# mmaker/c-lwe-snarks

Hardware: AMD Instinct MI355X
Metric: snark_proofs_per_sec (higher is better)
Workload: dtype u32 limbs (704-bit integers mod 2^704) + AES-256 bytes; int8 digits on the matrix cores, int32 accumulation (exact)

## Files before the change

c-lwe-snarks_amd/__init__.py:

```python
from __future__ import annotations

import ctypes
import os
from dataclasses import dataclass

import numpy as np

_HERE = os.path.dirname(os.path.abspath(__file__))
LIB_PATH = os.environ.get("MFHIP_LIB") or os.path.join(_HERE, "libmfhip.so")
P = 0xFFFFFFFB


class MfhError(RuntimeError):
    pass


@dataclass(frozen=True)
class Params:

    n: int = 1470
    logq: int = 736
    d: int = 1 << 15
    m: int = 21845

# ... 51 lines not shown
EXPORTS = [
    "mfh_ctx_create", "mfh_ctx_destroy", "mfh_set_stream", "mfh_sync", "mfh_scrub_staging", "mfh_last_error", "mfh_set_seed",
    "mfh_keystream", "mfh_sample_rows", "mfh_ct_add", "mfh_ct_mul_ui", "mfh_ct_addmul_ui", "mfh_eval_rows",
    "mfh_encrypt_rows", "mfh_decrypt", "mfh_ct_smudge", "mfh_ssp_upload", "mfh_witness_poly", "mfh_version",
    "mfh_workspace_bytes", "mfh_last_kernel_ms", "mfh_set_timing", "mfh_set_overlap", "mfh_eval_rows_multi", "mfh_prove_batch", "mfh_crs_mm_image_bytes", "mfh_crs_expand_mm", "mfh_crs_set_resident_mm", "mfh_witness_poly_multi", "mfh_witness_poly_mm", "mfh_poly_h_multi", "mfh_poly_mul", "mfh_poly_add", "mfh_poly_prepare_t",
    "mfh_ssp_prepare", "mfh_poly_h", "mfh_setup_messages", "mfh_setup", "mfh_setup_image", "mfh_crs_image_set_b", "mfh_prove",
    "mfh_prove_partial", "mfh_prove_finish", "mfh_ct_to_lanes", "mfh_ct_from_lanes", "mfh_lanes_per_value", "mfh_digest128", "mfh_timing_drain", "mfh_timing_busy_ms", "mfh_timing_work_rows", "mfh_set_batch_image", "mfh_set_batch_slabs", "mfh_set_expand_path", "mfh_set_expand_periods", "mfh_set_encrypt_path", "mfh_set_batch_launch", "mfh_set_batch_bw", "mfh_set_batch_witness", "mfh_witness_poly_stream", "mfh_set_mm_chunk_rows", "mfh_set_mm_pack", "mfh_set_poly_exact", "mfh_poly_exact_fallbacks", "mfh_poly_exact_points", "mfh_set_poly_exact_points", "mfh_set_mm_stream", "mfh_add_dotp", "mfh_set_encrypt_chunks", "mfh_set_witness_per", "mfh_set_eval_path", "mfh_set_decrypt_path", "mfh_decrypt_rows",
    "mfh_crs_mm_share_bytes", "mfh_crs_expand_mm_share", "mfh_crs_set_resident_mm_share", "mfh_batch_chain", "mfh_batch_witness_cols", "mfh_batch_chain_from_w", "mfh_witness_poly_mm_cols", "mfh_prove_batch_partial", "mfh_prove_batch_finish",
    "mfh_resident_row_bytes", "mfh_crs_expand", "mfh_eval_rows_resident", "mfh_crs_set_resident",
    "mfh_witness_lanes", "mfh_witness_from_lanes", "mfh_prove_partial_w", "mfh_verify",
    "mfh_ssp_set_prg", "mfh_ssp_prg_make_t", "mfh_ssp_prg_fill",
    "mfh_resident_share_rows", "mfh_crs_expand_share", "mfh_crs_set_resident_share", "mfh_crs_set_resident_prefix",
    "mfh_prove_batch_supergroup", "mfh_prove_batch_stream_wait", "mfh_set_mm_width", "mfh_set_mm_queue", "mfh_set_mm_claim_log", "mfh_mm_claim_log_launches",
    "mfh_setup_public", "mfh_prove_public", "mfh_prove_batch_public", "mfh_vk_derive", "mfh_verify_public",
    "mfh_ssp_from_rows", "mfh_ssp_set_rows", "mfh_ssp_rows_fill", "mfh_ssp_rows_violations", "mfh_circuit_create", "mfh_circuit_destroy", "mfh_circuit_assign",
    "mfh_circuit_create_global", "mfh_circuit_create_ex", "mfh_circuit_create_out", "mfh_circuit_create_sum",
    "mfh_merkle_create", "mfh_merkle_destroy", "mfh_merkle_set_leaves", "mfh_merkle_root", "mfh_merkle_nodes", "mfh_merkle_paths",
    "mfh_sha256_records", "mfh_merkle_set_records", "mfh_merkle_update_rows", "mfh_merkle_update_records",
    "mfh_merkle_absent_rows", "mfh_merkle_insert_keys", "mfh_merkle_update_rows_cut", "mfh_merkle_update_records_cut", "mfh_merkle_insert_keys_cut",
    "mfh_merkle_remove_keys", "mfh_merkle_remove_keys_cut", "mfh_merkle_transfer_keys", "mfh_merkle_transfer_keys_cut",
    "mfh_merkle_paths_cut", "mfh_merkle_absent_rows_cut", "mfh_merkle_range_rows", "mfh_merkle_range_rows_cut",
    "mfh_merkle_load_keys", "mfh_merkle_check_table", "mfh_merkle_grow", "mfh_merkle_grow_leaves",
    "mfh_merkle_write_keys", "mfh_merkle_write_keys_cut",
]


OPTIONAL_EXPORTS = {
    "mfh_set_mm_queue": "tuning knob; older builds walk fixed lists",
    "mfh_set_mm_claim_log": "test instrumentation of mfh_set_mm_queue",
    "mfh_mm_claim_log_launches": "test instrumentation of mfh_set_mm_queue",
    "mfh_set_expand_periods": "test knob; older builds pick the periods per chunk from the row count",
    "mfh_set_batch_witness": "tuning knob; older builds run the witness pass per super-group",
    "mfh_witness_poly_stream": "the streamed pass alone (tests); older builds have mfh_witness_poly_mm only",
}


def load_library():
    global _lib
    if _lib is not None:
        return _lib
    if not os.path.exists(LIB_PATH):
        raise MfhError(f"{LIB_PATH} is missing: run `python -c 'import __graft_entry__ as g; g.build()'` "
                       "(hipcc --offload-arch=gfx950).  There is no CPU fallback.")
    lib = ctypes.CDLL(LIB_PATH)
    vp, u64, sz, i32, u32 = ctypes.c_void_p, ctypes.c_uint64, ctypes.c_size_t, ctypes.c_int, ctypes.c_uint32
    sig = {
        "mfh_ctx_create": (i32, [ctypes.POINTER(vp), i32, ctypes.POINTER(_CParams)]),
        "mfh_ctx_destroy": (None, [vp]),
        "mfh_set_stream": (i32, [vp, vp]),
        "mfh_sync": (i32, [vp]),
        "mfh_scrub_staging": (i32, [vp]),
        "mfh_last_error": (ctypes.c_char_p, [vp]),
        "mfh_set_seed": (i32, [vp, ctypes.c_char_p]),
        "mfh_keystream": (i32, [vp, u64, vp, sz]),
        "mfh_sample_rows": (i32, [vp, u64, sz, vp]),
        "mfh_ct_add": (i32, [vp, vp, vp, vp, sz]),
# ... 48 lines not shown
        "mfh_ssp_set_prg": (i32, [vp, u64, vp]),
        "mfh_ssp_prg_make_t": (i32, [vp, u64, ctypes.c_char_p, vp]),
        "mfh_ssp_prg_fill": (i32, [vp, u64, sz, sz, vp]),
        "mfh_verify": (i32, [vp, vp, u32, u32, u32, vp, vp, sz, vp]),
        "mfh_witness_lanes": (i32, [vp, vp, ctypes.c_char_p, u32, u32, vp]),
        "mfh_witness_from_lanes": (i32, [vp, vp, vp, u32, vp]),
        "mfh_prove_partial_w": (i32, [vp, vp, vp, ctypes.c_char_p, u32, u32, u32, vp, vp]),
        "mfh_resident_row_bytes": (sz, [vp]),
        "mfh_crs_expand": (i32, [vp, u64, sz, vp, vp]),
        "mfh_crs_image_set_b": (i32, [vp, sz, sz, vp, vp]),
        "mfh_eval_rows_resident": (i32, [vp, vp, sz, sz, vp, vp, vp, vp, i32]),
        "mfh_crs_set_resident": (i32, [vp, vp]),
        "mfh_timing_drain": (i32, [vp, ctypes.c_char_p, ctypes.POINTER(u64), ctypes.POINTER(ctypes.c_double), ctypes.POINTER(u64),
                                   ctypes.POINTER(ctypes.c_float)]),
        "mfh_timing_busy_ms": (ctypes.c_double, [vp]),
        "mfh_timing_work_rows": (u64, [vp]),
        "mfh_set_batch_image": (i32, [vp, i32]),
        "mfh_set_mm_chunk_rows": (i32, [vp, u32]),
        "mfh_set_mm_pack": (i32, [vp, i32]),
        "mfh_set_poly_exact": (i32, [vp, i32]),
        "mfh_poly_exact_fallbacks": (ctypes.c_long, [vp]),
        "mfh_poly_exact_points": (i32, [vp, ctypes.POINTER(u32)]),
        "mfh_set_poly_exact_points": (i32, [vp, ctypes.POINTER(u32)]),
        "mfh_set_mm_stream": (i32, [vp, i32, i32, i32, u32]),
        "mfh_set_batch_launch": (i32, [vp, u32, i32]),
        "mfh_set_batch_bw": (i32, [vp, i32]),
        "mfh_set_batch_witness": (i32, [vp, i32]),
        "mfh_set_encrypt_path": (i32, [vp, i32]),
        "mfh_set_expand_path": (i32, [vp, i32]),
        "mfh_set_expand_periods": (i32, [vp, u32]),
        "mfh_set_batch_slabs": (i32, [vp, u32]),
        "mfh_set_encrypt_chunks": (i32, [vp, u32]),
        "mfh_set_eval_path": (i32, [vp, i32]),
        "mfh_set_decrypt_path": (i32, [vp, i32]),
        "mfh_decrypt_rows": (i32, [vp, u64, sz, vp, vp, vp]),
        "mfh_set_witness_per": (i32, [vp, u32]),
        "mfh_crs_mm_share_bytes": (sz, [vp, u32, u32]),
        "mfh_crs_expand_mm_share": (i32, [vp, vp, u32, u32, vp]),
        "mfh_crs_set_resident_mm_share": (i32, [vp, vp, u32, u32]),
        "mfh_batch_chain": (i32, [vp, vp, u32, ctypes.c_char_p, sz, vp, vp, vp, vp]),
        "mfh_batch_witness_cols": (i32, [vp, vp, u32, ctypes.c_char_p, sz, vp, u32, u32, vp, sz]),
        "mfh_batch_chain_from_w": (i32, [vp, vp, u32, vp, vp, vp]),
        "mfh_witness_poly_mm_cols": (i32, [vp, vp, u32, ctypes.c_char_p, sz, vp, u32, u32, vp, sz]),
        "mfh_prove_batch_partial": (i32, [vp, vp, u32, u32, u32, ctypes.c_char_p, sz, vp, vp, vp, sz, vp]),
        "mfh_prove_batch_finish": (i32, [vp, vp, u32, vp, ctypes.c_char_p, sz, ctypes.c_char_p, vp]),
        "mfh_setup_public": (i32, [vp, vp, u32, u32, u32, u32, vp, vp, vp, vp]),
# ... 951 lines not shown
    def set_mm_pack(self, on=True):
        self._chk(self.lib.mfh_set_mm_pack(self._h, 1 if on else 0))

    def set_poly_exact(self, mode=1):
        self._chk(self.lib.mfh_set_poly_exact(self._h, int(mode)))

    def poly_exact_fallbacks(self):
        return int(self.lib.mfh_poly_exact_fallbacks(self._h))

    def exact_points(self):
        out = (ctypes.c_uint32 * 4)()
        self._chk(self.lib.mfh_poly_exact_points(self._h, out))
        return [int(x) for x in out]

    def set_exact_points(self, pts):
        if pts is None:
            self._chk(self.lib.mfh_set_poly_exact_points(self._h, None))
            return
        pts = [int(x) for x in pts]
        if len(pts) != 4 or not all(0 <= x < 2**32 for x in pts):
            raise MfhError(f"set_exact_points: four uint32 values, got {pts!r}")
        self._chk(self.lib.mfh_set_poly_exact_points(self._h, (ctypes.c_uint32 * 4)(*pts)))

    def set_mm_chunk_rows(self, rows=0):
        self._chk(self.lib.mfh_set_mm_chunk_rows(self._h, int(rows)))

    def timing_drain(self, which):
        n, rows, ms, last = ctypes.c_uint64(), ctypes.c_uint64(), ctypes.c_double(), ctypes.c_float()
        self._chk(self.lib.mfh_timing_drain(self._h, which.encode(), ctypes.byref(n), ctypes.byref(ms), ctypes.byref(rows), ctypes.byref(last)))
        return n.value, ms.value, rows.value

    def timing_busy_ms(self):
        return float(self.lib.mfh_timing_busy_ms(self._h))

    def timing_work_rows(self):
        return int(self.lib.mfh_timing_work_rows(self._h))

    def last_kernel_ms(self, which):
        return float(self.lib.mfh_last_kernel_ms(self._h, which.encode()))

    def set_seed(self, seed: bytes):
        assert len(seed) == 40
        self._chk(self.lib.mfh_set_seed(self._h, bytes(seed)))

    def keystream(self, off, nbytes, out=None):
        out = self.empty(nbytes) if out is None else out
# ... 467 lines not shown
```

c-lwe-snarks_amd/csrc/ctx.hpp:

```cpp
#pragma once
#include <hip/hip_runtime.h>

#include <stdint.h>
#include <string.h>

#include <string>
#include <vector>

#include "aes_dev.hpp"
#include "batch_plan.hpp"
#include "mfhip.h"
#include "ssp_prg.hpp"

#define HIP_TRY(ctx, expr)                                                        \
  do {                                                                            \
    hipError_t e_ = (expr);                                                       \
    if (e_ != hipSuccess) {                                                       \
      (ctx)->err = std::string(#expr) + ": " + hipGetErrorString(e_);             \
      return MFH_EDEVICE;                                                         \
    }                                                                             \
  } while (0)

struct PolyState;
struct SspInterp;
// ... 65 lines not shown
  const uint32_t *ssp_frag_src = nullptr;
  DevBuf ssp_img;
  const uint32_t *ssp_img_src = nullptr;
  DevBuf wstream;
  hipEvent_t ev_wstage = nullptr, ev_wdigits = nullptr;
  int batch_witness = 1;
  SspInterp *interp = nullptr;
  DevBuf circ_io;
  DevBuf circ_state;
  DevBuf d_batch;
  DevBuf batch_img;
  int batch_image = 1;
  int mm_map = 1;
  bool mm_persist = true;
  bool mm_wave1 = false;
  uint32_t mm_sync_mode = 0, mm_spin = 64;
  uint32_t mm_width = 32;
  size_t early_ws_half = 0;
  bool batch_early_chain = false;
  uint32_t *mm_sync = nullptr;
  uint32_t mm_queue = 1, mm_queue_shift = 0; int mm_queue_prefix = -8;
  uint32_t *mm_log = nullptr; size_t mm_log_words = 0, mm_log_used = 0; uint32_t mm_log_n = 0, mm_log_desc[16][12];
  int poly_exact = 1;
  bool poly_pts_pinned = false;
  uint32_t poly_pts[4] = {0, 0, 0, 0};
  bool mm_pack = true;
  uint32_t mm_chunk_rows = 131071;
  int expand_path = 0;
  uint32_t expand_periods = 0;
  int enc_path = 0;
  uint32_t ncu = 256;
  int dec_path = 0;
  int eval_path = 0;
  uint32_t enc_chunks = 0;
  uint32_t witness_per = 0;
  uint32_t batch_slabs = 0;
  int batch_bw_merged = 1;
  int batch_merge = 1;
  uint32_t batch_ngl = 8;
  PinBuf pin_rows, pin_cw, pin_smudge;
  PinBuf pin_pub;
  DevBuf d_pub;
  PinBuf pin_wring[8];
  uint32_t pin_wnext = 0;
  hipEvent_t ev_sample = nullptr;
  DevBuf sample_tmp;
// ... 223 lines not shown
```

c-lwe-snarks_amd/csrc/poly.hip:

```cpp
#include <assert.h>
#include <errno.h>
#include <sys/syscall.h>
#include <unistd.h>

#include <algorithm>
#include <type_traits>

#include "ctx.hpp"
#include "ntt.hpp"

namespace {

#define MF_NEEDED(need, vs) do { if ((need) && (vs) >= *(need)) return; } while (0)

using namespace mf_ntt;

__device__ __forceinline__ uint32_t lz_mont(uint32_t a, uint32_t b, uint32_t p, uint32_t ninv) {
  uint64_t t = (uint64_t)a * b;
  uint32_t m = (uint32_t)t * ninv;
  return (uint32_t)((t + (uint64_t)m * p) >> 32);
}
__device__ __forceinline__ uint32_t lz_add(uint32_t a, uint32_t b, uint32_t p2) {
  uint32_t s = a + b;
  return min(s, s - p2);
// ... 282 lines not shown
#pragma unroll
  for (int m = 0; m < 8; m++) sm[lpad(8 * tid + m)] = v[m];
  __syncthreads();
#pragma unroll
  for (int m = 0; m < 8; m++) v[m] = sm[lpad(i3 + 4 * m)];
  dit_regs<3, true>(v, j3, 4, 8, ti, half_max, q);
#pragma unroll
  for (int m = 0; m < 8; m++) sm[lpad(i3 + 4 * m)] = v[m];
  __syncthreads();
#pragma unroll
  for (int m = 0; m < 8; m++) v[m] = sm[lpad(i2 + 32 * m)];
  dit_regs<3, true>(v, j2, 32, 64, ti, half_max, q);
#pragma unroll
  for (int m = 0; m < 8; m++) sm[lpad(i2 + 32 * m)] = v[m];
  __syncthreads();
#pragma unroll
  for (int m = 0; m < 8; m++) v[m] = sm[lpad(i1 + 256 * m)];
  dit_regs<3, true>(v, tid, 256, 512, ti, half_max, q);
#pragma unroll
  for (int m = 0; m < 8; m++) a[base + i1 + 256 * m] = lz_canon(v[m], q.p);
}

__global__ void k_crt(const uint32_t *__restrict__ r, uint32_t N, uint32_t count, Primes3 P, Crt C, uint32_t *__restrict__ out, size_t out_stride,
                      const uint32_t *__restrict__ need = nullptr, int64_t rev_top = -1, uint32_t nsrc = 0, const uint32_t *__restrict__ map = nullptr) {
  MF_NEEDED(need, blockIdx.y);
  uint32_t i = blockIdx.x * blockDim.x + threadIdx.x;
  if (i >= count) return;
  r += (size_t)blockIdx.y * 3 * N;
  out += (size_t)(map ? map[blockIdx.y] : blockIdx.y) * out_stride;
  if (rev_top < 0) {
    out[i] = crt_coeff(r[i], r[(size_t)N + i], r[(size_t)2 * N + i], P, C);
    return;
  }
  const int64_t e = rev_top - (int64_t)i;
  out[i] = e >= 0 && e < (int64_t)nsrc ? crt_coeff(r[e], r[(size_t)N + e], r[(size_t)2 * N + e], P, C) : 0u;
}
template <int K, bool LAST>
__global__ __launch_bounds__(256) void k_exact_seam(uint32_t *__restrict__ a, uint32_t N, const uint32_t *__restrict__ tw, const uint32_t *__restrict__ twi,
                                                    uint32_t half_max, Primes3 P, Crt C, uint32_t *__restrict__ out, uint32_t keep, size_t out_stride) {
  constexpr int R = 1 << K;
  constexpr uint32_t qd = 2048;
  const uint32_t j = blockIdx.x * blockDim.x + threadIdx.x;
  if (j >= qd || N != (qd << K)) return;
  uint32_t *x = a + (size_t)blockIdx.y * 3 * N + j;
  const NttPrime q1 = P.q[0], q2 = P.q[1], q3 = P.q[2];
  uint32_t r[R], x1[R], x2[R], cf[R];
#pragma unroll
  for (int m = 0; m < R; m++) r[m] = x[(size_t)m * qd];
  dit_regs<K>(r, j, qd, 2 * qd, twi, half_max, q1);
#pragma unroll
  for (int m = 0; m < R; m++) x1[m] = mont_mul(r[m], C.ninv_std[0], q1.p, q1.ninv);
  __builtin_amdgcn_sched_barrier(0);
#pragma unroll
  for (int m = 0; m < R; m++) r[m] = x[(size_t)N + (size_t)m * qd];
// ... 13 lines not shown
    const uint32_t x1m3 = x1[m] >= q3.p ? x1[m] - q3.p : x1[m], x2m3 = x2[m] >= q3.p ? x2[m] - q3.p : x2[m];
    const uint32_t t3 = mont_mul(sub_mod(r3, x1m3, q3.p), C.inv_p1_p3, q3.p, q3.ninv);
    const uint32_t x3 = mont_mul(sub_mod(t3, x2m3, q3.p), C.inv_p2_p3, q3.p, q3.ninv);
    cf[m] = red_p32((uint64_t)red_p32(x1[m]) + red_p32((uint64_t)x2[m] * C.p1_mod) + red_p32((uint64_t)x3 * C.p1p2_mod));
  }
  if (LAST) {
    out += (size_t)blockIdx.y * out_stride;
#pragma unroll
    for (int m = 0; m < R; m++)
      if (j + (uint32_t)m * qd < keep) out[j + (uint32_t)m * qd] = cf[m];
    return;
  }
  if (j == 0) cf[0] = cf[0] ? cf[0] - 1 : P32 - 1;
#pragma unroll
  for (int k = 0; k < 3; k++) {
    const NttPrime q = P.q[k];
#pragma unroll
    for (int m = 0; m < R; m++) r[m] = mont_mul(cf[m], q.r2, q.p, q.ninv);
    dif_regs<K>(r, j, qd, N, tw + (size_t)k * half_max, half_max, q);
#pragma unroll
    for (int m = 0; m < R; m++) x[(size_t)k * N + (size_t)m * qd] = lz_canon(r[m], q.p);
    __builtin_amdgcn_sched_barrier(0);
  }
}

__global__ void k_reverse(const uint32_t *__restrict__ in, int64_t top, uint32_t count, uint32_t *__restrict__ out, size_t in_stride = 0,
                          size_t out_stride = 0, const uint32_t *__restrict__ need = nullptr) {
  MF_NEEDED(need, blockIdx.y);
  uint32_t i = blockIdx.x * blockDim.x + threadIdx.x;
  if (i >= count) return;
  in += (size_t)blockIdx.y * in_stride;
  out += (size_t)blockIdx.y * out_stride;
  int64_t s = top - (int64_t)i;
  out[i] = s >= 0 ? in[s] : 0u;
}
__global__ void k_two_minus(uint32_t *__restrict__ e, uint32_t count) {
  uint32_t i = blockIdx.x * blockDim.x + threadIdx.x;
  if (i >= count) return;
  uint32_t v = e[i];
  uint32_t neg = v ? P32 - v : 0u;
  e[i] = i == 0 ? red_p32((uint64_t)neg + 2) : neg;
}
__global__ void k_sub_const0(uint32_t *__restrict__ a, uint32_t c, size_t stride = 0, const uint32_t *__restrict__ need = nullptr) {
  MF_NEEDED(need, blockIdx.x);
  if (threadIdx.x == 0) a[(size_t)blockIdx.x * stride] = red_p32((uint64_t)a[(size_t)blockIdx.x * stride] + P32 - c);
}
// ... 73 lines not shown

inline dim3 g1(uint32_t n) { return dim3((n + 255) / 256); }

}

struct PolyState {
  struct Words : DevBuf {
    operator uint32_t *() const { return as<uint32_t>(); }
  };
  Primes3 P{};
  uint32_t logmax = 0, half_max = 0;
  Words d_tw, d_twi;
  Words d_bufA, d_bufB;
  Words d_tmp, d_tmp2;
  uint32_t nb_cap = 0;
  bool have_t = false;
  uint32_t d = 0, dt = 0, n = 0, logN2 = 0;
  Words d_G;
  Words d_Ghat;
  Words d_f;
  bool cyc = false;
  uint32_t logNc = 0;
  Words d_That;
  Words d_chk;
  uint32_t chk_r[4]{};
  uint32_t chk_t[4]{};
  Words d_need;
  uint32_t *h_seen = nullptr;
  uint32_t rest = 0;
  ~PolyState() {
    for (Words *b : {&d_tw, &d_twi, &d_bufA, &d_bufB, &d_tmp, &d_tmp2, &d_G, &d_Ghat, &d_f, &d_That, &d_chk, &d_need}) dev_free(*b);
    if (h_seen) hipHostFree(h_seen);
  }
};

namespace {

const uint32_t kPrimes[3] = {998244353u, 897581057u, 880803841u};
const uint32_t kRoots[3] = {3u, 3u, 26u};
constexpr uint32_t kMaxBatch = 21845;

uint32_t to_mont(uint64_t x, const NttPrime &q) { return (uint32_t)(((unsigned __int128)(x % q.p) << 32) % q.p); }

int poly_batch_reserve(mfh_ctx *c, PolyState *S, uint32_t nb) {
  if (nb <= S->nb_cap) return MFH_OK;
  const size_t bytes = (size_t)nb * 4 << S->logmax;
  if (S->d_bufA.p) hipStreamSynchronize(c->stream);
  S->nb_cap = 0;
  for (PolyState::Words *b : {&S->d_bufA, &S->d_bufB, &S->d_tmp, &S->d_tmp2}) dev_free(*b);
  int rc = MFH_OK;
  for (PolyState::Words *b : {&S->d_bufA, &S->d_bufB})
    if (!rc) rc = dev_reserve(c, *b, 3 * bytes);
  for (PolyState::Words *b : {&S->d_tmp, &S->d_tmp2})
    if (!rc) rc = dev_reserve(c, *b, bytes);
// ... 206 lines not shown
  HIP_TRY(c, hipMemcpyAsync(&bottom, lev + off.back(), 4, hipMemcpyDeviceToHost, c->stream));
  HIP_TRY(c, hipStreamSynchronize(c->stream));
  if (!bottom) return MFH_OK;
  const uint32_t binv = invp(bottom);
  HIP_TRY(c, hipMemcpyAsync(inv[0], &binv, 4, hipMemcpyHostToDevice, c->stream));
  int cur = 0;
  for (int k = (int)off.size() - 2; k >= 0; k--) {
    const uint32_t n = Nc >> k;
    hipLaunchKernelGGL(k_conj, g1(n), dim3(256), 0, c->stream, lev + off[k], n, cj);
    hipLaunchKernelGGL(k_spread2, g1(n), dim3(256), 0, c->stream, inv[cur], n, sp);
    if ((rc = mul_tmp(cj, sp, n))) return rc;
    hipLaunchKernelGGL(k_fold, g1(n), dim3(256), 0, c->stream, S->d_tmp, n, inv[cur ^ 1]);
    cur ^= 1;
  }
  if ((rc = mul_tmp(lev, inv[cur], Nc))) return rc;
  hipLaunchKernelGGL(k_fold, g1(Nc), dim3(256), 0, c->stream, S->d_tmp, Nc, sp);
  std::vector<uint32_t> one(Nc);
  HIP_TRY(c, hipMemcpyAsync(one.data(), sp, (size_t)Nc * 4, hipMemcpyDeviceToHost, c->stream));
  HIP_TRY(c, hipStreamSynchronize(c->stream));
  if (one[0] != 1 || std::any_of(one.begin() + 1, one.end(), [](uint32_t x) { return x != 0; })) return MFH_OK;
  if ((rc = dev_reserve(c, S->d_That, (size_t)3 * Nc * 4))) return rc;
  ntt_load(c, S->d_That, Nc, 1, {inv[cur], Nc});
  ntt_blocks_forward(c, S->d_That, Nc, logNc, 1);
  std::vector<uint32_t> pw((size_t)4 * Nc);
  for (int j = 0, draws = 0; j < 4;) {
    uint32_t r = c->poly_pts[j];
    if (!c->poly_pts_pinned) {
      if (++draws > 64 || !draw_point(&r)) return MFH_OK;
      if (std::find(S->chk_r, S->chk_r + j, r) != S->chk_r + j) continue;
    }
    uint64_t x = 1, tv = 0;
    for (uint32_t i = 0; i < Nc; i++) {
      pw[(size_t)j * Nc + i] = (uint32_t)x;
      if (i < d) tv = (tv + x * t[i]) % P32;
      x = x * r % P32;
    }
    if (!tv && !c->poly_pts_pinned) continue;
    S->chk_r[j] = r;
    S->chk_t[j++] = (uint32_t)tv;
  }
  if ((rc = dev_reserve(c, S->d_chk, pw.size() * 4))) return rc;
  HIP_TRY(c, hipMemcpyAsync(S->d_chk, pw.data(), pw.size() * 4, hipMemcpyHostToDevice, c->stream));
  HIP_TRY(c, hipGetLastError());
  HIP_TRY(c, hipStreamSynchronize(c->stream));
  S->logNc = logNc;
  S->cyc = true;
// ... 38 lines not shown
    if (le < k2) HIP_TRY(c, hipMemsetAsync(S->d_tmp + le, 0, (size_t)(k2 - le) * 4, c->stream));
    hipLaunchKernelGGL(k_two_minus, g1(k2), dim3(256), 0, c->stream, S->d_tmp, k2);
    rc = poly_mul(c, {.a = S->d_G, .la = k, .b = S->d_tmp, .lb = k2, .out = S->d_tmp2, .keep = k2});
    if (rc) return rc;
    HIP_TRY(c, hipMemcpyAsync(S->d_G, S->d_tmp2, (size_t)k2 * 4, hipMemcpyDeviceToDevice, c->stream));
    k = k2;
  }
  return MFH_OK;
}

bool exact_policy(mfh_ctx *c, uint32_t nb) {
  PolyState *S = c->poly;
  if (!S->cyc || !c->poly_exact || nb < 4) return false;
  if (c->poly_exact != 1) return true;
  if (*(volatile uint32_t *)S->h_seen) {
    *(volatile uint32_t *)S->h_seen = 0;
    S->rest = 64;
  }
  if (!S->rest) return true;
  S->rest--;
  return false;
}

int h_exact(mfh_ctx *c, const uint32_t *d_v, uint32_t *d_h, uint32_t nb) {
  PolyState *S = c->poly;
  const uint32_t d = S->d, logNc = S->logNc, Nc = 1u << logNc;
  const size_t Nmax = (size_t)1 << S->logmax;
  HIP_TRY(c, hipMemsetAsync(S->d_need, 0, 4, c->stream));
  if (logNc >= 12 && logNc <= 16) {
    const Crt C = make_crt(S, logNc);
    const uint32_t K = logNc - 11;
    const dim3 gs(((Nc >> K) + 255) / 256, nb), gl(Nc >> 11, 3 * nb);
    auto product = [&](const uint32_t *bhat) {
      hipLaunchKernelGGL(k_ntt_lds_mul8, gl, dim3(256), 0, c->stream, S->d_bufA, bhat, Nc, S->d_tw, S->d_twi, S->half_max, S->P, (const uint32_t *)nullptr);
    };
    auto seam = [&](auto last, uint32_t *out, uint32_t keep, size_t stride) {
      with_stages(K, [&](auto k) {
        hipLaunchKernelGGL((k_exact_seam<k(), last()>), gs, dim3(256), 0, c->stream, S->d_bufA, Nc, S->d_tw, S->d_twi, S->half_max, S->P, C, out, keep, stride);
      });
    };
    ntt_top_passes(c, Ntt::forward, S->d_bufA, Nc, logNc, nb, nullptr, {d_v, d, d});
    product(nullptr);
    seam(std::false_type{}, nullptr, 0, 0);
    product(S->d_That);
    seam(std::true_type{}, d_h, d, d);
  } else {
    int rc = poly_mul(c, {.a = d_v, .la = d, .b = d_v, .lb = d, .out = S->d_tmp, .keep = Nc, .nb = nb, .in_stride = d, .out_stride = Nmax,
                          .log_cyc = logNc});
    if (rc) return rc;
    hipLaunchKernelGGL(k_sub_const0, dim3(nb), dim3(64), 0, c->stream, S->d_tmp, 1u, Nmax, (const uint32_t *)nullptr);
    rc = poly_mul(c, {.a = S->d_tmp, .la = Nc, .lb = Nc, .bhat = S->d_That, .log_hat = logNc, .out = d_h, .keep = d, .nb = nb, .in_stride = Nmax, .out_stride = d,
                      .log_cyc = logNc});
    if (rc) return rc;
  }
  hipLaunchKernelGGL(k_exact_check, dim3(nb), dim3(1024), 0, c->stream, d_v, d_h, d, S->d_chk, Nc, uint4{S->chk_t[0], S->chk_t[1], S->chk_t[2], S->chk_t[3]},
                     S->d_need, S->h_seen);
  return MFH_OK;
}

int h_euclid(mfh_ctx *c, const uint32_t *d_v, uint32_t *d_h, uint32_t nb, const uint32_t *need) {
  PolyState *S = c->poly;
  const uint32_t d = S->d, n = S->n;
  const size_t Nmax = (size_t)1 << S->logmax;
  const uint32_t *map = need ? need + 2 : nullptr;
  int rc;
  if (S->dt >= 1) {
    rc = poly_mul(c, {.a = d_v, .la = d, .b = d_v, .lb = d, .out = S->d_tmp2, .keep = n, .nb = nb, .in_stride = d, .out_stride = Nmax, .need = need, .a_map = map,
                      .rev_top = (int64_t)(2 * d - 2), .nsrc = 2 * d - 1});
    if (rc) return rc;
    rc = poly_mul(c, {.a = S->d_tmp2, .la = n, .lb = n, .bhat = S->d_Ghat, .log_hat = S->logN2, .out = d_h, .keep = d, .nb = nb, .in_stride = Nmax, .out_stride = d,
                      .need = need, .out_map = map, .rev_top = (int64_t)n - 1, .nsrc = n});
    if (rc) return rc;
  } else {
    rc = poly_mul(c, {.a = d_v, .la = d, .b = d_v, .lb = d, .out = S->d_tmp, .keep = 2 * d - 1, .nb = nb, .in_stride = d, .out_stride = Nmax, .need = need,
                      .a_map = map});
    if (rc) return rc;
    hipLaunchKernelGGL(k_sub_const0, dim3(nb), dim3(64), 0, c->stream, S->d_tmp, 1u, Nmax, need);
// ... 56 lines not shown
  ntt_load(c, S->d_Ghat, N2, 1, {S->d_G, n});
  ntt_blocks_forward(c, S->d_Ghat, N2, S->logN2, 1);
  HIP_TRY(c, hipGetLastError());
  HIP_TRY(c, hipStreamSynchronize(c->stream));
  if ((rc = prepare_exact(c, d_t, t))) return rc;
  S->have_t = true;
  return MFH_OK;
}

int mfh_poly_h_multi(mfh_ctx *c, const uint32_t *d_v, uint32_t *d_h, uint32_t nb) {
  if (!c || !d_v || !d_h || !nb || nb > kMaxBatch) return MFH_EINVAL;
  PolyState *S = c->poly;
  if (!S || !S->have_t) {
    c->err = "mfh_poly_prepare_t has not been called for this SSP";
    return MFH_EINVAL;
  }
  HIP_TRY(c, hipSetDevice(c->device));
  int rc = poly_batch_reserve(c, S, nb);
  if (rc) return rc;
  const bool exact = exact_policy(c, nb);
  if (exact && (rc = h_exact(c, d_v, d_h, nb))) return rc;
  return h_euclid(c, d_v, d_h, nb, exact ? (const uint32_t *)S->d_need : nullptr);
}
int mfh_set_poly_exact(mfh_ctx *c, int mode) {
  if (!c || mode < 0 || mode > 2) return MFH_EINVAL;
  c->poly_exact = mode;
  if (c->poly && c->poly->h_seen) {
    *c->poly->h_seen = 0;
    c->poly->rest = 0;
  }
  return MFH_OK;
}
long mfh_poly_exact_fallbacks(mfh_ctx *c) {
  if (!c || !c->poly || !c->poly->cyc) return -1;
  HIP_TRY(c, hipSetDevice(c->device));
  uint32_t w[2] = {0, 0};
  if (hipMemcpyAsync(w, c->poly->d_need, 8, hipMemcpyDeviceToHost, c->stream) != hipSuccess || hipStreamSynchronize(c->stream) != hipSuccess ||
      hipMemsetAsync(c->poly->d_need + 1, 0, 4, c->stream) != hipSuccess)
    return -1;
  return (long)w[1];
}
int mfh_poly_exact_points(mfh_ctx *c, uint32_t *out) {
  if (!c || !out || !c->poly || !c->poly->have_t || !c->poly->cyc) return MFH_EINVAL;
  std::copy(c->poly->chk_r, c->poly->chk_r + 4, out);
  return MFH_OK;
}
// ... 24 lines not shown
```

c-lwe-snarks_amd/host/mfuoco_gpu.c:

```c
#define _GNU_SOURCE
#include <errno.h>
#include <pthread.h>
#include <stdbool.h>
#include <stdio.h>
#include <stdlib.h>
#include <string.h>
#include <strings.h>
#include <sys/random.h>
#include <unistd.h>

#include <gmp.h>

#define __HIP_PLATFORM_AMD__ 1
#include <hip/hip_runtime_api.h>

#include "mfhip.h"
#include "mfuoco/mangiafuoco_api.h"

#define L_LIMBS 12
#define K_LIMBS 11
#define CTL ((size_t)(GAMMA_N + 1) * L_LIMBS)
#define PIN_BYTES ((size_t)4 << 20)
#define ENC_CHUNK ((size_t)16384)
#define ENC_UP ((size_t)L_LIMBS * 8 + 4)
// ... 183 lines not shown
}

static bool shim_warm_on(void)
{
  const char *e = getenv("MFUOCO_GPU_WARM");
  return !(e && *e && !atoi(e));
}
static mfh_ctx *gpu(void)
{
  if (G.ctx) return G.ctx;
  if (G.device < 0) {
    const char *e = getenv("MFUOCO_GPU");
    G.device = e ? atoi(e) : 0;
  }
  mfh_params P = { GAMMA_N, GAMMA_LOGQ, (uint32_t)GAMMA_D, (uint32_t)GAMMA_M };
  if (mfh_ctx_create(&G.ctx, G.device, &P) != MFH_OK) {
    fprintf(stderr, "libmfuoco_gpu: no usable HIP device %d (there is no CPU fallback)\n", G.device);
    abort();
  }
  CK(mfh_set_stream(G.ctx, NULL));
  {
    const char *e = getenv("MFUOCO_GPU_POLY_EXACT");
    if (e && *e && atoi(e) >= 0 && atoi(e) <= 2) CK(mfh_set_poly_exact(G.ctx, atoi(e)));
  }
  size_t rows = 2 * (size_t)GAMMA_D + GAMMA_M;
  for (int i = 0; i < 3; i++) HK(hipMalloc((void **)&G.d_ct[i], CTL * 8 + 256));
  HK(hipMalloc((void **)&G.d_sk, (size_t)GAMMA_N * L_LIMBS * 8));
  HK(hipMalloc((void **)&G.d_c8, rows * CT_BYTES));
  HK(hipMalloc((void **)&G.d_co, rows * 4));
  HK(hipMalloc((void **)&G.d_proof, 5 * CTL * 8));
  HK(hipMalloc((void **)&G.d_crs, rows * CT_BYTES));
  HK(hipHostMalloc((void **)&G.pin, PIN_BYTES, hipHostMallocDefault));
  HK(hipEventCreateWithFlags(&G.ev_small, hipEventDisableTiming));
  HK(hipEventCreateWithFlags(&G.ev_img, hipEventDisableTiming));
  HK(hipStreamCreateWithFlags(&G.s2, hipStreamNonBlocking));
  HK(hipHostMalloc((void **)&G.pin_sk, (size_t)GAMMA_N * L_LIMBS * 8, hipHostMallocDefault));
  G.h_sk = xcalloc((size_t)GAMMA_N * L_LIMBS, 8);
  if (shim_warm_on()) {
    static const uint8_t zero_seed[40];
    CK(mfh_set_seed(G.ctx, zero_seed));
    HK(hipMemset(G.d_c8, 0, (size_t)GAMMA_D * CT_BYTES));
    HK(hipMemset(G.d_co, 1, (size_t)GAMMA_D * 4));
    CK(mfh_eval_rows(G.ctx, 0, GAMMA_D, G.d_c8, G.d_co, NULL, G.d_ct[2], NULL, 0));
    CK(mfh_sync(G.ctx));
    memset(G.pin, 0, (size_t)1 << 20);
    HK(hipMemcpy(G.d_c8, G.pin, (size_t)1 << 20 < rows * CT_BYTES ? (size_t)1 << 20 : rows * CT_BYTES, hipMemcpyHostToDevice));
// ... 1229 lines not shown
```

include/mfhip.h:

```cpp
#pragma once
#include <stddef.h>
#include <stdint.h>

#ifdef __cplusplus
extern "C" {
#endif

#define MFH_P 0xfffffffbu

enum {
  MFH_OK = 0,
  MFH_EINVAL = -1,
  MFH_EDEVICE = -2,
  MFH_ENOMEM = -3,
  MFH_EUNSUPPORTED = -4
};

typedef struct {
  uint32_t n;
  uint32_t logq;
  uint32_t d;
  uint32_t m;
} mfh_params;

// ... 152 lines not shown
                              uint32_t field_hi, uint32_t nk, const uint8_t *h_keys, size_t key_stride, const uint8_t *h_values, size_t value_stride,
                              const uint8_t *h_expect, size_t expect_stride, uint32_t ncuts, const uint32_t *h_cuts, uint8_t *const *h_rows,
                              const size_t *h_strides, uint8_t *h_roots, uint32_t *h_index, uint8_t *h_status);
int mfh_merkle_balance_sum(mfh_ctx *ctx, const mfh_merkle *t, const uint8_t *d_table, size_t table_stride, uint32_t length, uint32_t key_bytes,
                           uint32_t amount_bytes, uint64_t h_sum[2], uint32_t *h_live);
int mfh_merkle_load_keys(mfh_ctx *ctx, mfh_merkle *t, uint8_t *d_table, size_t table_stride, uint32_t length, uint32_t key_bytes, uint32_t nk,
                         const uint8_t *d_keys, const uint8_t *d_payloads, uint32_t payload_bytes, uint32_t h_status[3]);
int mfh_merkle_check_table(mfh_ctx *ctx, const mfh_merkle *t, const uint8_t *d_table, size_t table_stride, uint32_t length, uint32_t key_bytes,
                           uint32_t h_out[4]);
int mfh_merkle_grow(mfh_ctx *ctx, const mfh_merkle *t, uint32_t new_depth, const uint8_t *d_table, size_t table_stride, uint32_t length,
                    uint8_t *d_new_table, size_t new_stride, mfh_merkle **out, uint8_t *h_roots);
int mfh_merkle_grow_leaves(mfh_ctx *ctx, const mfh_merkle *t, uint32_t new_depth, mfh_merkle **out, uint8_t *h_roots);

int mfh_poly_mul(mfh_ctx *ctx, const uint32_t *d_a, size_t la, const uint32_t *d_b, size_t lb, uint32_t *d_c);
int mfh_poly_add(mfh_ctx *ctx, const uint32_t *d_a, const uint32_t *d_b, size_t count, uint32_t *d_out);
int mfh_poly_prepare_t(mfh_ctx *ctx, const uint32_t *d_t);
int mfh_ssp_prepare(mfh_ctx *ctx, const uint32_t *d_ssp);
int mfh_poly_h(mfh_ctx *ctx, const uint32_t *d_v, uint32_t *d_h);
int mfh_poly_h_multi(mfh_ctx *ctx, const uint32_t *d_v, uint32_t *d_h, uint32_t nb);
int mfh_set_poly_exact(mfh_ctx *ctx, int mode);
long mfh_poly_exact_fallbacks(mfh_ctx *ctx);
int mfh_poly_exact_points(mfh_ctx *ctx, uint32_t *out);
int mfh_set_poly_exact_points(mfh_ctx *ctx, const uint32_t *pts);

int mfh_setup_messages(mfh_ctx *ctx, const uint32_t *d_ssp, uint32_t alpha, uint32_t beta, uint32_t s, uint32_t *d_msg);
int mfh_setup(mfh_ctx *ctx, const uint32_t *d_ssp, uint32_t alpha, uint32_t beta, uint32_t s, const uint64_t *d_sk,
              const uint64_t *d_err, uint8_t *d_crs_c8);
int mfh_setup_image(mfh_ctx *ctx, const uint32_t *d_ssp, uint32_t alpha, uint32_t beta, uint32_t s, const uint64_t *d_sk,
                    const uint64_t *d_err, uint8_t *d_crs_c8, void *d_rows_image);
int mfh_prove(mfh_ctx *ctx, const uint8_t *d_crs_c8, const uint32_t *d_ssp, const uint8_t *h_witness_bits, uint32_t delta,
              const uint8_t *h_smudge_mag, size_t maglen, const uint8_t *h_smudge_sign, uint64_t *d_proof);

int mfh_verify(mfh_ctx *ctx, const uint32_t *d_ssp, uint32_t alpha, uint32_t beta, uint32_t s, const uint64_t *d_sk,
               const uint64_t *d_proofs, size_t count, uint8_t *d_ok);

int mfh_setup_public(mfh_ctx *ctx, const uint32_t *d_ssp, uint32_t alpha, uint32_t beta, uint32_t s, uint32_t lu, const uint64_t *d_sk,
                     const uint64_t *d_err, uint8_t *d_crs_c8, void *d_rows_image);
int mfh_prove_public(mfh_ctx *ctx, const uint8_t *d_crs_c8, const uint32_t *d_ssp, uint32_t lu, const uint8_t *h_bits, uint32_t delta,
                     const uint8_t *h_smudge_mag, size_t maglen, const uint8_t *h_smudge_sign, uint64_t *d_proof);
int mfh_prove_batch_public(mfh_ctx *ctx, const uint8_t *d_crs_c8, const uint32_t *d_ssp, uint32_t lu, uint32_t nproofs, const uint8_t *h_bits,
                           size_t bits_stride, const uint32_t *h_delta, const uint8_t *h_smudge_mag, size_t maglen, const uint8_t *h_smudge_sign,
                           uint64_t *d_proofs);
int mfh_vk_derive(mfh_ctx *ctx, const uint32_t *d_ssp, uint32_t s, uint32_t lu, uint32_t *d_vk);
int mfh_verify_public(mfh_ctx *ctx, const uint32_t *d_vk, uint32_t lu, uint32_t alpha, uint32_t beta, const uint64_t *d_sk, const uint64_t *d_proofs,
                      const uint8_t *h_statements, size_t stmt_stride, size_t count, uint8_t *d_ok);

// ... 74 lines not shown
```

Before: 14690.

## Compute cyclic quotient with single-block LDS NTT kernel for 2^15 size

Adds a k_cyc_lds kernel that, for a cyclic length of 2^15, performs the forward NTT, pointwise product and inverse NTT for one prime inside one 1024-thread workgroup. The three radix-32 passes exchange data through LDS instead of launching separate global-memory layer and seam kernels. Twiddle tables are precomputed per layer and the hat of t is transposed into a layout that matches the kernel. The subtract-one step is folded into the CRT kernel. This is meant to remove several launches and global round trips in the exact-division h computation. In exchange each transform runs on only 3*nb workgroups, so parallelism is limited when the batch is small.

```diff
diff --git a/c-lwe-snarks_amd/__init__.py b/c-lwe-snarks_amd/__init__.py
--- a/c-lwe-snarks_amd/__init__.py
+++ b/c-lwe-snarks_amd/__init__.py
@@ -97,6 +97,7 @@
     "mfh_merkle_paths_cut", "mfh_merkle_absent_rows_cut", "mfh_merkle_range_rows", "mfh_merkle_range_rows_cut",
     "mfh_merkle_load_keys", "mfh_merkle_check_table", "mfh_merkle_grow", "mfh_merkle_grow_leaves",
     "mfh_merkle_write_keys", "mfh_merkle_write_keys_cut",
+    "mfh_set_poly_lds", "mfh_poly_h_cyclic",
 ]
 
 
@@ -107,6 +108,8 @@
     "mfh_set_expand_periods": "test knob; older builds pick the periods per chunk from the row count",
     "mfh_set_batch_witness": "tuning knob; older builds run the witness pass per super-group",
     "mfh_witness_poly_stream": "the streamed pass alone (tests); older builds have mfh_witness_poly_mm only",
+    "mfh_set_poly_lds": "A/B knob; older builds multiply through the seam kernels",
+    "mfh_poly_h_cyclic": "the cyclic quotient alone (tests)",
 }
 
 
@@ -201,6 +204,8 @@
         "mfh_poly_exact_fallbacks": (ctypes.c_long, [vp]),
         "mfh_poly_exact_points": (i32, [vp, ctypes.POINTER(u32)]),
         "mfh_set_poly_exact_points": (i32, [vp, ctypes.POINTER(u32)]),
+        "mfh_set_poly_lds": (i32, [vp, i32]),
+        "mfh_poly_h_cyclic": (i32, [vp, vp, u32, vp]),
         "mfh_set_mm_stream": (i32, [vp, i32, i32, i32, u32]),
         "mfh_set_batch_launch": (i32, [vp, u32, i32]),
         "mfh_set_batch_bw": (i32, [vp, i32]),
@@ -1198,6 +1203,15 @@
             raise MfhError(f"set_exact_points: four uint32 values, got {pts!r}")
         self._chk(self.lib.mfh_set_poly_exact_points(self._h, (ctypes.c_uint32 * 4)(*pts)))
 
+    def set_poly_lds(self, on=True):
+        self._chk(self.lib.mfh_set_poly_lds(self._h, 1 if on else 0))
+
+    def poly_h_cyclic(self, d_v, nb):
+        N = 1 << max(self.params.d - 1, 1).bit_length()
+        out = self.empty(nb * N * 4)
+        self._chk(self.lib.mfh_poly_h_cyclic(self._h, _ptr(d_v), nb, _ptr(out)))
+        return out
+
     def set_mm_chunk_rows(self, rows=0):
         self._chk(self.lib.mfh_set_mm_chunk_rows(self._h, int(rows)))
 
diff --git a/c-lwe-snarks_amd/csrc/ctx.hpp b/c-lwe-snarks_amd/csrc/ctx.hpp
--- a/c-lwe-snarks_amd/csrc/ctx.hpp
+++ b/c-lwe-snarks_amd/csrc/ctx.hpp
@@ -111,6 +111,7 @@
   uint32_t mm_queue = 1, mm_queue_shift = 0; int mm_queue_prefix = -8;
   uint32_t *mm_log = nullptr; size_t mm_log_words = 0, mm_log_used = 0; uint32_t mm_log_n = 0, mm_log_desc[16][12];
   int poly_exact = 1;
+  int poly_lds = 1;
   bool poly_pts_pinned = false;
   uint32_t poly_pts[4] = {0, 0, 0, 0};
   bool mm_pack = true;
diff --git a/c-lwe-snarks_amd/csrc/poly.hip b/c-lwe-snarks_amd/csrc/poly.hip
--- a/c-lwe-snarks_amd/csrc/poly.hip
+++ b/c-lwe-snarks_amd/csrc/poly.hip
@@ -328,14 +328,16 @@
 }
 
 __global__ void k_crt(const uint32_t *__restrict__ r, uint32_t N, uint32_t count, Primes3 P, Crt C, uint32_t *__restrict__ out, size_t out_stride,
-                      const uint32_t *__restrict__ need = nullptr, int64_t rev_top = -1, uint32_t nsrc = 0, const uint32_t *__restrict__ map = nullptr) {
+                      const uint32_t *__restrict__ need = nullptr, int64_t rev_top = -1, uint32_t nsrc = 0, const uint32_t *__restrict__ map = nullptr,
+                      uint32_t sub0 = 0) {
   MF_NEEDED(need, blockIdx.y);
   uint32_t i = blockIdx.x * blockDim.x + threadIdx.x;
   if (i >= count) return;
   r += (size_t)blockIdx.y * 3 * N;
   out += (size_t)(map ? map[blockIdx.y] : blockIdx.y) * out_stride;
   if (rev_top < 0) {
-    out[i] = crt_coeff(r[i], r[(size_t)N + i], r[(size_t)2 * N + i], P, C);
+    const uint32_t x = crt_coeff(r[i], r[(size_t)N + i], r[(size_t)2 * N + i], P, C);
+    out[i] = i == 0 && sub0 ? (x ? x - 1 : P32 - 1) : x;
     return;
   }
   const int64_t e = rev_top - (int64_t)i;
@@ -395,6 +397,97 @@
     for (int m = 0; m < R; m++) x[(size_t)k * N + (size_t)m * qd] = lz_canon(r[m], q.p);
     __builtin_amdgcn_sched_barrier(0);
   }
+}
+
+constexpr uint32_t kLdsLog = 15, kLdsN = 1u << kLdsLog;
+__device__ __forceinline__ void dif_layers(uint32_t *v, uint32_t j, uint32_t qd, int s0, const uint32_t *__restrict__ lay, const NttPrime q) {
+#pragma unroll
+  for (int st = 0; st < 5; st++) {
+    const int h = 16 >> st;
+    const uint32_t *l = lay + (kLdsN - (kLdsN >> (s0 + st)));
+#pragma unroll
+    for (int m = 0; m < 32; m++)
+      if ((m & h) == 0) lz_dif(v[m], v[m + h], l[j + (uint32_t)(m & (h - 1)) * qd], q.p, q.ninv);
+    __builtin_amdgcn_sched_barrier(0);
+  }
+}
+__device__ __forceinline__ void dit_layers(uint32_t *v, uint32_t j, uint32_t qd, int s0, const uint32_t *__restrict__ lay, const NttPrime q) {
+#pragma unroll
+  for (int st = 0; st < 5; st++) {
+    const int h = 1 << st;
+    const uint32_t *l = lay + (kLdsN - (kLdsN >> (s0 + 4 - st)));
+#pragma unroll
+    for (int m = 0; m < 32; m++)
+      if ((m & h) == 0) lz_dit(v[m], v[m + h], l[j + (uint32_t)(m & (h - 1)) * qd], q.p, q.ninv);
+    __builtin_amdgcn_sched_barrier(0);
+  }
+}
+__global__ __launch_bounds__(1024) void k_cyc_lds(const uint32_t *__restrict__ in, uint32_t in_len, size_t in_stride, const uint32_t *__restrict__ bhat_t,
+                                                  const uint32_t *__restrict__ lay, const uint32_t *__restrict__ layi, Primes3 P, uint32_t *__restrict__ out) {
+  __shared__ uint32_t sm[kLdsN + kLdsN / 32];
+  const uint32_t tid = threadIdx.x, k = blockIdx.y % 3;
+  const NttPrime q = P.q[k];
+  const uint32_t *src = in + (size_t)(blockIdx.y / 3) * in_stride;
+  const uint32_t *t = lay + (size_t)k * kLdsN, *ti = layi + (size_t)k * kLdsN;
+  const uint32_t j2 = tid & 31;
+  uint32_t *s1 = sm + lpad(tid), *s2 = sm + lpad((tid >> 5) * 1024 + j2), *s3 = sm + 33 * tid;
+  uint32_t v[32];
+#pragma unroll
+  for (int m = 0; m < 32; m++) {
+    const uint32_t e = tid + 1024u * m;
+    v[m] = e < in_len ? mont_mul(src[e], q.r2, q.p, q.ninv) : 0u;
+  }
+  dif_layers(v, tid, 1024, 0, t, q);
+#pragma unroll
+  for (int m = 0; m < 32; m++) s1[1056 * m] = v[m];
+  __syncthreads();
+#pragma unroll
+  for (int m = 0; m < 32; m++) v[m] = s2[33 * m];
+  dif_layers(v, j2, 32, 5, t, q);
+#pragma unroll
+  for (int m = 0; m < 32; m++) s2[33 * m] = v[m];
+  __syncthreads();
+#pragma unroll
+  for (int m = 0; m < 32; m++) v[m] = s3[m];
+  dif_layers(v, 0, 1, 10, t, q);
+  if (bhat_t) {
+    const uint32_t *bp = bhat_t + (size_t)k * kLdsN + tid;
+#pragma unroll
+    for (int m = 0; m < 32; m++) v[m] = lz_mont(v[m], bp[1024 * m], q.p, q.ninv);
+  } else {
+#pragma unroll
+    for (int m = 0; m < 32; m++) v[m] = lz_mont(v[m], v[m], q.p, q.ninv);
+  }
+  dit_layers(v, 0, 1, 10, ti, q);
+#pragma unroll
+  for (int m = 0; m < 32; m++) s3[m] = v[m];
+  __syncthreads();
+#pragma unroll
+  for (int m = 0; m < 32; m++) v[m] = s2[33 * m];
+  dit_layers(v, j2, 32, 5, ti, q);
+#pragma unroll
+  for (int m = 0; m < 32; m++) s2[33 * m] = v[m];
+  __syncthreads();
+#pragma unroll
+  for (int m = 0; m < 32; m++) v[m] = s1[1056 * m];
+  dit_layers(v, tid, 1024, 0, ti, q);
+  uint32_t *dst = out + (size_t)blockIdx.y * kLdsN + tid;
+#pragma unroll
+  for (int m = 0; m < 32; m++) dst[1024 * m] = lz_canon(v[m], q.p);
+}
+__global__ void k_lds_layers(const uint32_t *__restrict__ tw, const uint32_t *__restrict__ twi, uint32_t half_max, uint32_t *__restrict__ lay) {
+  const uint32_t e = blockIdx.x * blockDim.x + threadIdx.x;
+  if (e >= kLdsN) return;
+  uint32_t s = 0;
+  while (s < kLdsLog && e >= kLdsN - (kLdsN >> (s + 1))) s++;
+  const uint32_t i = e - (kLdsN - (kLdsN >> s));
+  const uint32_t *src = (blockIdx.z ? twi : tw) + (size_t)blockIdx.y * half_max;
+  lay[((size_t)blockIdx.z * 3 + blockIdx.y) * kLdsN + e] = s < kLdsLog ? src[(size_t)(i << s) * (half_max * 2 / kLdsN)] : 0u;
+}
+__global__ void k_lds_hat_t(const uint32_t *__restrict__ hat, uint32_t *__restrict__ out) {
+  const uint32_t e = blockIdx.x * blockDim.x + threadIdx.x;
+  if (e >= kLdsN) return;
+  out[(size_t)blockIdx.y * kLdsN + e] = hat[(size_t)blockIdx.y * kLdsN + 32 * (e & 1023) + (e >> 10)];
 }
 
 __global__ void k_reverse(const uint32_t *__restrict__ in, int64_t top, uint32_t count, uint32_t *__restrict__ out, size_t in_stride = 0,
@@ -514,6 +607,7 @@
   bool cyc = false;
   uint32_t logNc = 0;
   Words d_That;
+  Words d_ThatT, d_lay;
   Words d_chk;
   uint32_t chk_r[4]{};
   uint32_t chk_t[4]{};
@@ -521,7 +615,7 @@
   uint32_t *h_seen = nullptr;
   uint32_t rest = 0;
   ~PolyState() {
-    for (Words *b : {&d_tw, &d_twi, &d_bufA, &d_bufB, &d_tmp, &d_tmp2, &d_G, &d_Ghat, &d_f, &d_That, &d_chk, &d_need}) dev_free(*b);
+    for (Words *b : {&d_tw, &d_twi, &d_bufA, &d_bufB, &d_tmp, &d_tmp2, &d_G, &d_Ghat, &d_f, &d_That, &d_ThatT, &d_lay, &d_chk, &d_need}) dev_free(*b);
     if (h_seen) hipHostFree(h_seen);
   }
 };
@@ -774,6 +868,11 @@
   if ((rc = dev_reserve(c, S->d_That, (size_t)3 * Nc * 4))) return rc;
   ntt_load(c, S->d_That, Nc, 1, {inv[cur], Nc});
   ntt_blocks_forward(c, S->d_That, Nc, logNc, 1);
+  if (logNc == kLdsLog) {
+    if ((rc = dev_reserve(c, S->d_ThatT, (size_t)3 * Nc * 4)) || (rc = dev_reserve(c, S->d_lay, (size_t)6 * Nc * 4))) return rc;
+    hipLaunchKernelGGL(k_lds_hat_t, dim3(Nc / 256, 3), dim3(256), 0, c->stream, S->d_That, S->d_ThatT);
+    hipLaunchKernelGGL(k_lds_layers, dim3(Nc / 256, 3, 2), dim3(256), 0, c->stream, S->d_tw, S->d_twi, S->half_max, S->d_lay);
+  }
   std::vector<uint32_t> pw((size_t)4 * Nc);
   for (int j = 0, draws = 0; j < 4;) {
     uint32_t r = c->poly_pts[j];
@@ -858,12 +957,25 @@
   return false;
 }
 
-int h_exact(mfh_ctx *c, const uint32_t *d_v, uint32_t *d_h, uint32_t nb) {
+int h_cyclic(mfh_ctx *c, const uint32_t *d_v, uint32_t nb, uint32_t *d_out, uint32_t keep, size_t out_stride) {
   PolyState *S = c->poly;
   const uint32_t d = S->d, logNc = S->logNc, Nc = 1u << logNc;
   const size_t Nmax = (size_t)1 << S->logmax;
-  HIP_TRY(c, hipMemsetAsync(S->d_need, 0, 4, c->stream));
-  if (logNc >= 12 && logNc <= 16) {
+  if (logNc == kLdsLog && c->poly_lds) {
+    const Crt C = make_crt(S, logNc);
+    const uint32_t *lay = S->d_lay;
+    auto product = [&](const uint32_t *in, uint32_t len, size_t stride, const uint32_t *bhat_t) {
+      hipLaunchKernelGGL(k_cyc_lds, dim3(1, 3 * nb), dim3(1024), 0, c->stream, in, len, stride, bhat_t, lay, lay + (size_t)3 * Nc, S->P, (uint32_t *)S->d_bufA);
+    };
+    auto coeffs = [&](uint32_t *out, uint32_t count, size_t stride, uint32_t sub0) {
+      hipLaunchKernelGGL(k_crt, dim3((count + 255) / 256, nb), dim3(256), 0, c->stream, S->d_bufA, Nc, count, S->P, C, out, stride, (const uint32_t *)nullptr,
+                         (int64_t)-1, 0u, (const uint32_t *)nullptr, sub0);
+    };
+    product(d_v, d, d, nullptr);
+    coeffs(S->d_tmp, Nc, Nmax, 1u);
+    product(S->d_tmp, Nc, Nmax, S->d_ThatT);
+    coeffs(d_out, keep, out_stride, 0u);
+  } else if (logNc >= 12 && logNc <= 16) {
     const Crt C = make_crt(S, logNc);
     const uint32_t K = logNc - 11;
     const dim3 gs(((Nc >> K) + 255) / 256, nb), gl(Nc >> 11, 3 * nb);
@@ -879,16 +991,26 @@
     product(nullptr);
     seam(std::false_type{}, nullptr, 0, 0);
     product(S->d_That);
-    seam(std::true_type{}, d_h, d, d);
+    seam(std::true_type{}, d_out, keep, out_stride);
   } else {
     int rc = poly_mul(c, {.a = d_v, .la = d, .b = d_v, .lb = d, .out = S->d_tmp, .keep = Nc, .nb = nb, .in_stride = d, .out_stride = Nmax,
                           .log_cyc = logNc});
     if (rc) return rc;
     hipLaunchKernelGGL(k_sub_const0, dim3(nb), dim3(64), 0, c->stream, S->d_tmp, 1u, Nmax, (const uint32_t *)nullptr);
-    rc = poly_mul(c, {.a = S->d_tmp, .la = Nc, .lb = Nc, .bhat = S->d_That, .log_hat = logNc, .out = d_h, .keep = d, .nb = nb, .in_stride = Nmax, .out_stride = d,
-                      .log_cyc = logNc});
+    rc = poly_mul(c, {.a = S->d_tmp, .la = Nc, .lb = Nc, .bhat = S->d_That, .log_hat = logNc, .out = d_out, .keep = keep, .nb = nb, .in_stride = Nmax,
+                      .out_stride = out_stride, .log_cyc = logNc});
     if (rc) return rc;
   }
+  HIP_TRY(c, hipGetLastError());
+  return MFH_OK;
+}
+
+int h_exact(mfh_ctx *c, const uint32_t *d_v, uint32_t *d_h, uint32_t nb) {
+  PolyState *S = c->poly;
+  const uint32_t d = S->d, Nc = 1u << S->logNc;
+  HIP_TRY(c, hipMemsetAsync(S->d_need, 0, 4, c->stream));
+  const int rc = h_cyclic(c, d_v, nb, d_h, d, d);
+  if (rc) return rc;
   hipLaunchKernelGGL(k_exact_check, dim3(nb), dim3(1024), 0, c->stream, d_v, d_h, d, S->d_chk, Nc, uint4{S->chk_t[0], S->chk_t[1], S->chk_t[2], S->chk_t[3]},
                      S->d_need, S->h_seen);
   return MFH_OK;
@@ -991,6 +1113,23 @@
   if (exact && (rc = h_exact(c, d_v, d_h, nb))) return rc;
   return h_euclid(c, d_v, d_h, nb, exact ? (const uint32_t *)S->d_need : nullptr);
 }
+int mfh_poly_h_cyclic(mfh_ctx *c, const uint32_t *d_v, uint32_t nb, uint32_t *d_out) {
+  if (!c || !d_v || !d_out || !nb || nb > kMaxBatch) return MFH_EINVAL;
+  PolyState *S = c->poly;
+  if (!S || !S->have_t || !S->cyc) {
+    c->err = "mfh_poly_h_cyclic: no t prepared, or it has no exact-division path";
+    return MFH_EINVAL;
+  }
+  HIP_TRY(c, hipSetDevice(c->device));
+  const int rc = poly_batch_reserve(c, S, nb);
+  if (rc) return rc;
+  return h_cyclic(c, d_v, nb, d_out, 1u << S->logNc, (size_t)1 << S->logNc);
+}
+int mfh_set_poly_lds(mfh_ctx *c, int on) {
+  if (!c) return MFH_EINVAL;
+  c->poly_lds = on ? 1 : 0;
+  return MFH_OK;
+}
 int mfh_set_poly_exact(mfh_ctx *c, int mode) {
   if (!c || mode < 0 || mode > 2) return MFH_EINVAL;
   c->poly_exact = mode;
diff --git a/c-lwe-snarks_amd/host/mfuoco_gpu.c b/c-lwe-snarks_amd/host/mfuoco_gpu.c
--- a/c-lwe-snarks_amd/host/mfuoco_gpu.c
+++ b/c-lwe-snarks_amd/host/mfuoco_gpu.c
@@ -229,6 +229,8 @@
   {
     const char *e = getenv("MFUOCO_GPU_POLY_EXACT");
     if (e && *e && atoi(e) >= 0 && atoi(e) <= 2) CK(mfh_set_poly_exact(G.ctx, atoi(e)));
+    e = getenv("MFUOCO_GPU_POLY_LDS");
+    if (e && *e) CK(mfh_set_poly_lds(G.ctx, atoi(e) != 0));
   }
   size_t rows = 2 * (size_t)GAMMA_D + GAMMA_M;
   for (int i = 0; i < 3; i++) HK(hipMalloc((void **)&G.d_ct[i], CTL * 8 + 256));
diff --git a/include/mfhip.h b/include/mfhip.h
--- a/include/mfhip.h
+++ b/include/mfhip.h
@@ -198,6 +198,8 @@
 long mfh_poly_exact_fallbacks(mfh_ctx *ctx);
 int mfh_poly_exact_points(mfh_ctx *ctx, uint32_t *out);
 int mfh_set_poly_exact_points(mfh_ctx *ctx, const uint32_t *pts);
+int mfh_set_poly_lds(mfh_ctx *ctx, int on);
+int mfh_poly_h_cyclic(mfh_ctx *ctx, const uint32_t *d_v, uint32_t nb, uint32_t *d_out);
 
 int mfh_setup_messages(mfh_ctx *ctx, const uint32_t *d_ssp, uint32_t alpha, uint32_t beta, uint32_t s, uint32_t *d_msg);
 int mfh_setup(mfh_ctx *ctx, const uint32_t *d_ssp, uint32_t alpha, uint32_t beta, uint32_t s, const uint64_t *d_sk,
```

After: 14790, median of 6. About the same (+0.7%).
